# joeyee/Onet

Hardware: AMD Instinct MI355X
Metric: training images/sec (twin 256x256 pass) (higher is better)
Workload: dtype f32

## Files before the change

### onet_amd/_lib.py

```python
from __future__ import annotations

import ctypes
import os
import re

HERE = os.path.dirname(os.path.abspath(__file__))
HEADER = os.path.join(os.path.dirname(HERE), "include", "onet_hip.h")
EVAL_HEADER = os.path.join(os.path.dirname(HERE), "include", "onet_hip_eval.h")
RAGGED_HEADER = os.path.join(os.path.dirname(HERE), "include", "onet_hip_ragged.h")
RAGGED_SPLIT_HEADER = os.path.join(os.path.dirname(HERE), "include", "onet_hip_ragged_split.h")
LIBPATH = os.environ.get("ONET_HIP_LIB") or os.path.join(HERE, "libonet_hip.so")

_CT = {
    "int": ctypes.c_int,
    "int64_t": ctypes.c_int64,
    "uint64_t": ctypes.c_uint64,
    "float": ctypes.c_float,
    "double": ctypes.c_double,
}


def parse_header(path: str = HEADER):
    src = open(path).read()
    src = re.sub(r"/\*.*?\*/", " ", src, flags=re.S)
    src = re.sub(r"//[^\n]*", " ", src)
    src = re.sub(r"^\s*#.*$", " ", src, flags=re.M)
    protos = {}
    for m in re.finditer(r"((?:const\s+)?\w+\s*\*?)\s*(onet_\w+)\s*\(([^)]*)\)\s*;", src):
        ret, name, args = m.group(1).strip(), m.group(2), m.group(3).strip()
        if ret.endswith("*"):
            restype = ctypes.c_char_p if "char" in ret else ctypes.c_void_p
        else:
            restype = _CT[ret]
        argtypes, argnames = [], []
        if args and args != "void":
            for a in args.split(","):
                a = a.strip()
                mm = re.match(r"(?:const\s+)?(\w+)\s*(\*?)\s*(\w+)$", a)
                if not mm:
                    raise ValueError(f"cannot parse argument {a!r} of {name}")
                base, ptr, an = mm.groups()
                argtypes.append(ctypes.c_void_p if ptr else _CT[base])
                argnames.append(an)
        protos[name] = (restype, argtypes, argnames)
    return protos


class OnetHipError(RuntimeError):
    pass


_lib = None
_protos = None


def load(build_if_missing: bool = True):
    global _lib, _protos
    if _lib is not None:
        return _lib
    if not os.path.exists(LIBPATH):
        if not build_if_missing:
            raise OnetHipError(f"{LIBPATH} not built; run `python -m onet_amd.build`")
        from . import build as _build
        _build.build()
    lib = ctypes.CDLL(LIBPATH)
    _protos = {}
    for header in (HEADER, EVAL_HEADER, RAGGED_HEADER, RAGGED_SPLIT_HEADER):
        protos = parse_header(header)
        for name, (restype, argtypes, _) in protos.items():
            try:
                fn = getattr(lib, name)
            except AttributeError as e:
                raise OnetHipError(f"libonet_hip.so does not export {name} declared in {os.path.basename(header)}") from e
            fn.restype = restype
            fn.argtypes = argtypes
        _protos.update(protos)
    _lib = lib
    return lib


def last_error() -> str:
    return load().onet_last_error().decode()


PROFILE_HOOK = None


def call(name: str, *args, nbytes=None):
    lib = load()
    hook = PROFILE_HOOK
    tok = hook.begin() if hook is not None else None
    rc = getattr(lib, name)(*args)
    if tok is not None:
        hook.end(name, nbytes, tok)
    if rc != 0:
        raise OnetHipError(f"{name} failed ({rc}): {lib.onet_last_error().decode()}")
    return rc
```

### onet_amd/build.py

```python
import os
import subprocess
import sys

HERE = os.path.dirname(os.path.abspath(__file__))
CSRC = os.path.join(HERE, "csrc")
LIB = os.path.join(HERE, "libonet_hip.so")
SOURCES = ["abi.cpp", "conv_mfma.hip", "conv_wino4.hip", "conv_wino4w.hip", "conv_split.hip", "convt_gemm.hip", "stem.hip", "bn.hip", "spatial.hip", "head_loss.hip", "optim.hip", "evalside.hip", "clutter.hip"]
ARCH = "gfx950"


def _stale():
    if not os.path.exists(LIB):
        return True
    t = os.path.getmtime(LIB)
    deps = [os.path.join(CSRC, f) for f in os.listdir(CSRC) if f.endswith((".hip", ".cpp", ".hpp"))] + \
        [os.path.join(HERE, "..", "include", h) for h in ("onet_hip.h", "onet_hip_eval.h", "onet_hip_ragged.h", "onet_hip_ragged_split.h")]
    return any(os.path.getmtime(d) > t for d in deps)


def build(force=False, verbose=False, variant=None, flags=()):
    lib = LIB if variant is None else os.path.join(HERE, f"libonet_hip_{variant}.so")
    if variant is None and not force and not _stale():
        return LIB
    hipcc = os.environ.get("HIPCC", "/opt/rocm/bin/hipcc")
    objdir = CSRC if variant is None else os.path.join(CSRC, "_" + variant)
    os.makedirs(objdir, exist_ok=True)
    objs = []
    procs = []
    for src in SOURCES:
        obj = os.path.join(objdir, src.rsplit(".", 1)[0] + ".o")
        cmd = [hipcc, "-x", "hip", f"--offload-arch={ARCH}", "-O3", "-fPIC", "-std=c++17", "-Wall",
               "-Wno-unused-result", "-fno-slp-vectorize", *flags, "-c", os.path.join(CSRC, src), "-o", obj]
        if verbose:
            cmd.insert(-4, "-Rpass-analysis=kernel-resource-usage")
        procs.append((src, subprocess.Popen(cmd, stdout=subprocess.PIPE, stderr=subprocess.STDOUT, text=True)))
        objs.append(obj)
    failed = False
    for src, p in procs:
        out, _ = p.communicate()
        if p.returncode != 0:
            failed = True
            sys.stderr.write(f"[onet_amd.build] {src} failed:\n{out}\n")
        elif verbose or out.strip():
            sys.stderr.write(out)
    if failed:
        raise RuntimeError("hipcc failed building libonet_hip.so")
    subprocess.check_call([hipcc, "-shared", "-fPIC", f"--offload-arch={ARCH}", "-o", lib] + objs)
    return lib

# ... 8 lines not shown
```

### onet_amd/csrc/conv_split.hip

```cpp
#include <algorithm>
#include <cstdlib>
#include "common.hpp"
#include "../../include/onet_hip_ragged.h"
#include "../../include/onet_hip_ragged_split.h"

using namespace onet;

typedef float f32x16 __attribute__((ext_vector_type(16)));
typedef __bf16 bf16x8 __attribute__((ext_vector_type(8)));
typedef __bf16 bf16x2 __attribute__((ext_vector_type(2)));
typedef unsigned int u32x4s __attribute__((ext_vector_type(4)));
typedef float f32x4s __attribute__((ext_vector_type(4)));

namespace {

constexpr unsigned OOB_S = 0x80000000u;

__device__ __forceinline__ __amdgpu_buffer_rsrc_t s_rsrc(const void* base, int64_t bytes) {
    const int n = bytes > 0x7fffffffll ? 0x7fffffff : (int)bytes;
    return __builtin_amdgcn_make_buffer_rsrc(const_cast<void*>(base), 0, n, 0x00020000);
}
__device__ __forceinline__ void split2(float a, float b, unsigned& hi, unsigned& mid) {
    const bf16x2 h = {(__bf16)a, (__bf16)b};
    const bf16x2 m = {(__bf16)(a - (float)h[0]), (__bf16)(b - (float)h[1])};
    hi = __builtin_bit_cast(unsigned, h);
    mid = __builtin_bit_cast(unsigned, m);
}

typedef _Float16 f16x2 __attribute__((ext_vector_type(2)));
typedef _Float16 f16x8 __attribute__((ext_vector_type(8)));
__device__ __forceinline__ unsigned pack2bf(float lo, float hi) {
    const bf16x2 v = {(__bf16)lo, (__bf16)hi};
    return __builtin_bit_cast(unsigned, v);
}
__device__ __forceinline__ void split2h(float a, float b, unsigned& hi, unsigned& mid) {
    const f16x2 h = {(_Float16)a, (_Float16)b};
    const f16x2 m = {(_Float16)(a - (float)h[0]), (_Float16)(b - (float)h[1])};
    hi = __builtin_bit_cast(unsigned, h);
    mid = __builtin_bit_cast(unsigned, m);
}

__global__ void absmax_slots_kernel(const float* __restrict__ v, int64_t n, unsigned* __restrict__ slots) {
    float m = 0.f;
    for (int64_t i = blockIdx.x * (int64_t)blockDim.x + threadIdx.x; i < n; i += (int64_t)gridDim.x * blockDim.x) m = fmaxf(m, fabsf(v[i]));
#pragma unroll
    for (int o = 32; o > 0; o >>= 1) m = fmaxf(m, __shfl_xor(m, o, 64));
    if ((threadIdx.x & 63) == 0)
        atomicMax(slots + ((blockIdx.x * (blockDim.x >> 6) + (threadIdx.x >> 6)) & (AMAX_SLOTS - 1)) * AMAX_STRIDE, __builtin_bit_cast(unsigned, m));
}

__global__ void pack3x3_split_kernel(const float* __restrict__ w, __bf16* __restrict__ wq, int Cout, int Cin, int which, int f16,
                                     const unsigned* __restrict__ wamax) {
    const int K = which == 0 ? Cin : ((Cout + 15) / 16) * 16, N = which == 0 ? Cout : Cin;
    const int64_t n = (int64_t)K * 9 * N;
    const int nparts = f16 == 2 ? 1 : 2;
    float winv = 1.f;
    const float wscale = f16 == 1 ? amax_scale(amax_read(wamax), true, winv) : 1.f;
    if (blockIdx.x == 0 && threadIdx.x == 0) {
        float* meta = reinterpret_cast<float*>(wq + nparts * n);
        meta[0] = wscale;
        meta[1] = winv;
    }
    for (int64_t i = blockIdx.x * (int64_t)blockDim.x + threadIdx.x; i < n; i += (int64_t)gridDim.x * blockDim.x) {
        const int kc = (int)(i & 7);
        int64_t r = i >> 3;
        const int nn = (int)(r % N);
        r /= N;
        const int half = (int)(r & 1);
        r >>= 1;
        const int t = (int)(r % 9), kg = (int)(r / 9);
        const int k = kg * 16 + half * 8 + kc;
        float v = 0.f;
        if (which == 0) v = w[((int64_t)nn * Cin + k) * 9 + t];
        else if (k < Cout) v = w[((int64_t)k * Cin + nn) * 9 + (8 - t)];
        const int64_t per_chunk_part = (int64_t)9 * 2 * N * 8;
        const int64_t within = i - (int64_t)kg * per_chunk_part;
        if (f16 == 2) {
            wq[(int64_t)kg * per_chunk_part + within] = (__bf16)v;
        } else if (f16) {
            _Float16* wh = reinterpret_cast<_Float16*>(wq);
            const float vs = v * wscale;
            const _Float16 hi = (_Float16)vs;
            wh[((int64_t)kg * 2 + 0) * per_chunk_part + within] = hi;
            wh[((int64_t)kg * 2 + 1) * per_chunk_part + within] = (_Float16)(vs - (float)hi);
        } else {
            const __bf16 hi = (__bf16)v;
            wq[((int64_t)kg * 2 + 0) * per_chunk_part + within] = hi;
            wq[((int64_t)kg * 2 + 1) * per_chunk_part + within] = (__bf16)(v - (float)hi);
        }
    }
}

struct SpArgs {
    const float* x;
    int64_t x_bs;
    const __bf16* wq;
    float* z;
    int64_t z_bs;
    int B, Cin, Cout, H, W, tilesX, tilesY, coTiles;
    float* stats;
    const float* nsave;
    int nimg;
    const unsigned* x_amax;
    int x_always;
};

#define ONET_SP_DPP_ADD(v, ctrl, rmask) \
    v += __builtin_bit_cast(float, __builtin_amdgcn_update_dpp(0, __builtin_bit_cast(int, v), ctrl, rmask, 0xf, false))
__device__ __forceinline__ float sp_half_sum(float v) {
    ONET_SP_DPP_ADD(v, 0x128, 0xf);
    ONET_SP_DPP_ADD(v, 0x124, 0xf);
    ONET_SP_DPP_ADD(v, 0x122, 0xf);
    ONET_SP_DPP_ADD(v, 0x121, 0xf);
    ONET_SP_DPP_ADD(v, 0x142, 0xa);
    return v;
}
#undef ONET_SP_DPP_ADD

struct SpCfg {
    static constexpr int NW = 8, NT = 2, TW = 32, CO_T = 64;
    static constexpr int ROWS = NW * NT;
    static constexpr int IN_ROWS = ROWS + 2, IN_COLS = TW + 2;
    static constexpr int NPIX = IN_ROWS * IN_COLS;
// ... 2105 lines not shown
#undef ONET_SWP_LAUNCH
    int rc = check_launch("conv3x3_split_wgrad_pre_kernel");
    if (rc) return rc;
    return launch_wgrad_reduce((const float*)ws, dw, a.splitK * slabs, 9, Cout, Cin, 0, accumulate, as_stream(stream));
}

int onet_conv3x3_split_pack_weights(const float* w, void* wq_fwd, void* wq_dgrad, void* amax_ws, int Cout, int Cin, int fwd_f16,
                                    int dgrad_f16, void* stream) {
    ONET_REQUIRE(w && (wq_fwd || wq_dgrad), "conv3x3_split_pack_weights: null pointer");
    ONET_REQUIRE(amax_ws || !(fwd_f16 == 1 || dgrad_f16 == 1), "conv3x3_split_pack_weights: the fp16 packs need the 8 KB magnitude workspace");
    if (fwd_f16 == 1 || dgrad_f16 == 1) {
        (void)hipMemsetAsync(amax_ws, 0, AMAX_SLOTS * AMAX_STRIDE * sizeof(unsigned), as_stream(stream));
        const int64_t nw = (int64_t)Cout * Cin * 9;
        hipLaunchKernelGGL(absmax_slots_kernel, dim3((unsigned)std::min<int64_t>((nw + 1023) / 1024, 1024)), dim3(256), 0, as_stream(stream), w,
                           nw, (unsigned*)amax_ws);
        int rc0 = check_launch("absmax_slots_kernel");
        if (rc0) return rc0;
    }
    ONET_REQUIRE(Cout > 0 && Cin > 0, "conv3x3_split_pack_weights: bad shape");
    ONET_REQUIRE(!wq_fwd || (Cin % 16) == 0, "conv3x3_split_pack_weights: the forward pack needs Cin %% 16 == 0");
    const int64_t n = (int64_t)std::max(Cin, ((Cout + 15) / 16) * 16) * 9 * std::max(Cin, Cout);
    const int blocks = (int)std::min<int64_t>((n + 255) / 256, 8192);
    if (wq_fwd) {
        hipLaunchKernelGGL(pack3x3_split_kernel, dim3(blocks), dim3(256), 0, as_stream(stream), w, (__bf16*)wq_fwd, Cout, Cin, 0, fwd_f16,
                           (const unsigned*)amax_ws);
        int rc = check_launch("pack3x3_split_kernel");
        if (rc) return rc;
    }
    if (wq_dgrad) hipLaunchKernelGGL(pack3x3_split_kernel, dim3(blocks), dim3(256), 0, as_stream(stream), w, (__bf16*)wq_dgrad, Cout, Cin, 1,
                                     dgrad_f16, (const unsigned*)amax_ws);
    return check_launch("pack3x3_split_kernel");
}

int onet_conv3x3_split_fwd(const float* x, int64_t x_bs, const void* wq, int wq_f16, float* z, int64_t z_bs, int B, int Cin, int Cout,
                           int H, int W, void* stream) {
    return split_fwd(x, x_bs, wq, z, z_bs, B, Cin, Cout, H, W, stream, nullptr, wq_f16);
}

int onet_absmax_slots(const float* x, int64_t n, void* slots, void* stream) {
    ONET_REQUIRE(x && slots && n > 0, "absmax_slots: bad args");
    hipLaunchKernelGGL(absmax_slots_kernel, dim3((unsigned)std::min<int64_t>((n + 1023) / 1024, 4096)), dim3(256), 0, as_stream(stream), x, n,
                       (unsigned*)slots);
    return check_launch("absmax_slots_kernel");
}

int onet_conv3x3_split_conv_amax(const float* x, int64_t x_bs, const void* x_amax, int scale_always, const void* wq, float* z, int64_t z_bs,
                                 float* part, int B, int Cin, int Cout, int H, int W, void* stream) {
    return split_fwd(x, x_bs, wq, z, z_bs, B, Cin, Cout, H, W, stream, part, 1, nullptr, 0, (const unsigned*)x_amax, scale_always);
}

int onet_conv3x3_split_wgrad_f16(const float* x, int64_t x_bs, const void* x_amax, const float* save, int n_groups, const float* dz,
                                 int64_t dz_bs, const void* dz_amax, float* dw, void* ws, int64_t ws_bytes, int B, int Cin, int Cout,
                                 int H, int W, int accumulate, void* stream) {
    return split_wgrad_impl(x, x_bs, dz, dz_bs, dw, ws, ws_bytes, B, Cin, Cout, H, W, accumulate, stream, save, save ? n_groups : 0, 1,
                            (const unsigned*)x_amax, (const unsigned*)dz_amax);
}

int onet_conv3x3_split_fwd_norm(const float* z_prev, int64_t z_bs, const float* save, int n_groups, const void* wq, int wq_f16,
                                const void* x_amax, float* z, int64_t zo_bs, float* part, int B, int Cin, int Cout, int H, int W,
                                void* stream) {
    ONET_REQUIRE(save, "conv3x3_split_fwd_norm: null pointer");
    return split_fwd(z_prev, z_bs, wq, z, zo_bs, B, Cin, Cout, H, W, stream, part, wq_f16, save, n_groups, (const unsigned*)x_amax);
}

int onet_split_pack_act(const float* x, int64_t x_bs, void* xs, int64_t xs_bs, int B, int C, int H, int W, int f16, float scale,
                        const void* slots, void* stream) {
// ... 395 lines not shown
```

### onet_amd/csrc/convt_gemm.hip

```cpp
#include <algorithm>
#include <cstdlib>
#include "common.hpp"
#include "../../include/onet_hip_ragged.h"
#include "../../include/onet_hip_ragged_split.h"

using namespace onet;

typedef float f32x16 __attribute__((ext_vector_type(16)));
typedef float f32x4g __attribute__((ext_vector_type(4)));
typedef float f32x2g __attribute__((ext_vector_type(2)));
typedef int i32x4g __attribute__((ext_vector_type(4)));
typedef __bf16 bf16x8g __attribute__((ext_vector_type(8)));
typedef __bf16 bf16x2g __attribute__((ext_vector_type(2)));
typedef unsigned u32x4g __attribute__((ext_vector_type(4)));

namespace {

__device__ __forceinline__ i32x4g g_rsrc(const void* base, int64_t bytes) {
    const uint64_t p = reinterpret_cast<uint64_t>(base);
    i32x4g r;
    r.x = (int)(p & 0xffffffffu);
    r.y = (int)((p >> 32) & 0xffffu);
    r.z = bytes > 0x7fffffffll ? 0x7fffffff : (int)bytes;
    r.w = 0x00020000;
    return r;
}
__device__ __forceinline__ unsigned g_lds(const float* p) {
    return (unsigned)(uintptr_t)(__attribute__((address_space(3))) const float*)p;
}
__device__ __forceinline__ void g_dma16(i32x4g rsrc, unsigned lds_base, unsigned voff) {
    unsigned keep;
    asm volatile("s_nop 4\n\ts_mov_b32 %0, m0\n\ts_mov_b32 m0, %3\n\ts_nop 0\n\tbuffer_load_dwordx4 %1, %2, 0 offen lds\n\ts_mov_b32 m0, %0"
                 : "=&s"(keep)
                 : "v"(voff), "s"(rsrc), "s"(lds_base)
                 : "memory");
// ... 932 lines not shown
    }

    float undo = 1.f, dy_inv = 1.f;
    if constexpr (NP == 2) {
        float x_inv;
        (void)amax_scale(amax_read(g.x_slots), false, x_inv);
        (void)amax_scale(amax_read(g.dy_slots), true, dy_inv);
        undo = x_inv * dy_inv;
    }
    float* slab = g.slab + (int64_t)ks * g.Cin * 4 * g.Ct;
#pragma unroll
    for (int t = 0; t < TM; ++t)
#pragma unroll
        for (int u = 0; u < 2; ++u) {
            const int col = (GB * 8 * nt + chf * 32 + l31) * 4 + 2 * di + u;
#pragma unroll
            for (int r = 0; r < 16; ++r) {
                const int ci = C::MT * mt + wr * (TM * 32) + t * 32 + (r & 3) + 8 * (r >> 2) + 4 * kh;
                slab[(int64_t)ci * 4 * g.Ct + col] = acc[t][u][r] * undo;
            }
        }
    if (bias_wave && kh == 0) {
#pragma unroll
        for (int u = 0; u < 2; ++u) g.db_part[((int64_t)ks * 4 + 2 * di + u) * g.Ct + GB * 8 * nt + chf * 32 + l31] = accb[u][0] * dy_inv;
    }
}

__global__ void convt_pack_slots_kernel(const float* __restrict__ w, void* __restrict__ wP, void* __restrict__ wdP, int Cin, int Ct, int np,
                                        const unsigned* __restrict__ wamax) {
    const int M = 4 * Ct;
    const int64_t n = (int64_t)Cin * M;
    float winv = 1.f;
    const float wscale = np == 2 ? amax_scale(amax_read(wamax), true, winv) : 1.f;
    if (np == 2 && blockIdx.x == 0 && threadIdx.x == 0) {
        float* meta = reinterpret_cast<float*>(reinterpret_cast<_Float16*>(wP) + 2 * n);
        meta[0] = wscale;
        meta[1] = winv;
        if (wdP) {
            float* md = reinterpret_cast<float*>(reinterpret_cast<_Float16*>(wdP) + 2 * n);
            md[0] = wscale;
            md[1] = winv;
        }
    }
    for (int64_t i2 = blockIdx.x * (int64_t)blockDim.x + threadIdx.x; i2 < (wdP ? 2 * n : n); i2 += (int64_t)gridDim.x * blockDim.x) {
        if (i2 >= n) {
            const int64_t i = i2 - n;
            const int kc = (int)(i & 7);
            const int64_t r = i >> 3;
            const int ci = (int)(r % Cin), ks = (int)(r / Cin);
            const int c = (ks >> 2) * 8 + kc, q = ks & 3;
            const float v = w[((int64_t)ci * Ct + c) * 4 + q];
            if (np == 2) {
                _Float16* o = reinterpret_cast<_Float16*>(wdP);
                const float vs = v * wscale;
                const _Float16 hi = (_Float16)vs;
                o[(((int64_t)ks * 2 + 0) * Cin + ci) * 8 + kc] = hi;
                o[(((int64_t)ks * 2 + 1) * Cin + ci) * 8 + kc] = (_Float16)(vs - (float)hi);
            } else {
                reinterpret_cast<__bf16*>(wdP)[((int64_t)ks * Cin + ci) * 8 + kc] = (__bf16)v;
            }
            continue;
        }
        const int64_t i = i2;
        const int kc = (int)(i & 7);
        const int64_t r = i >> 3;
        const int m = (int)(r % M), c8 = (int)(r / M);
        const float v = w[(int64_t)(c8 * 8 + kc) * M + m];
        if (np == 2) {
            _Float16* o = reinterpret_cast<_Float16*>(wP);
            const float vs = v * wscale;
            const _Float16 hi = (_Float16)vs;
            o[(((int64_t)c8 * 2 + 0) * M + m) * 8 + kc] = hi;
            o[(((int64_t)c8 * 2 + 1) * M + m) * 8 + kc] = (_Float16)(vs - (float)hi);
        } else {
            reinterpret_cast<__bf16*>(wP)[((int64_t)c8 * M + m) * 8 + kc] = (__bf16)v;
        }
    }
}

__global__ void convt_absmax_kernel(const float* __restrict__ x, int64_t n, unsigned* __restrict__ slots) {
    float m = 0.f;
    for (int64_t i = blockIdx.x * (int64_t)blockDim.x + threadIdx.x; i < n; i += (int64_t)gridDim.x * blockDim.x) m = fmaxf(m, fabsf(x[i]));
#pragma unroll
    for (int o = 32; o > 0; o >>= 1) m = fmaxf(m, __shfl_xor(m, o, 64));
    if ((threadIdx.x & 63) == 0 && m == m)
        atomicMax(slots + ((blockIdx.x * (blockDim.x >> 6) + (threadIdx.x >> 6)) & (AMAX_SLOTS - 1)) * AMAX_STRIDE, __builtin_bit_cast(unsigned, m));
}

bool aligned16(const void* p) { return (reinterpret_cast<uintptr_t>(p) & 15) == 0; }

void wgrad_plan(int B, int Cin, int Ct, int h, int w, int& splitK, int& per) {
    const int64_t chunks = (int64_t)B * h * w / KP;
    const int64_t tiles = (int64_t)(Cin / 128) * (Ct / 32);
    int64_t k = std::max<int64_t>(1, (512 + tiles - 1) / tiles);
    k = std::min<int64_t>(k, std::max<int64_t>(1, chunks / 16));
    k = std::min<int64_t>(k, std::max<int64_t>(1, (256ll << 20) / ((int64_t)Cin * 4 * Ct * 4)));
    per = (int)((chunks + k - 1) / k);
    splitK = (int)((chunks + per - 1) / per);
}

}

namespace onet {


int convt_gemm_fwd(const float* x, int64_t x_bs, const float* wq, const float* bias, float* y, int64_t y_bs, void* y16, int64_t y16_bs,
                   int B, int Cin, int Ct, int h, int w, int Ho, int Wo, int pt, int pl, int prec, hipStream_t st, int y16_split,
                   const void* out_slots) {
    const int64_t hw = (int64_t)h * w;
    if (pt || pl || Ho != 2 * h || Wo != 2 * w || (Cin % KC) || (Ct % 32) || (hw % 128) || (w & 1) || !aligned16(x) || !aligned16(wq) ||
// ... 250 lines not shown
```

### onet_amd/ops.py

```python
from __future__ import annotations

import torch

from . import _lib

F32 = torch.float32


import os as _os


def _flags_from_env():
    out = {}
    for item in _os.environ.get("ONET_FLAGS", "").split(","):
        if "=" in item:
            k, v = item.split("=", 1)
            out[k.strip()] = v.strip()
    return out


_FLAGS = _flags_from_env()


def _flag(name, default):
# ... 322 lines not shown
    Cin, Cout = w.shape[0], w.shape[1]
    wq = torch.empty(Cin * 4 * Cout, dtype=F32, device=w.device)
    _lib.call("onet_convT2x2_pack_weights_fused", _p(w), _p(wq), Cin, Cout, _stream())
    return wq


CONVT_BF16 = _flag("CONVT_BF16", True)


def convT2x2_fwd(x, wq, bias, out, Ct, pt, pl):
    require_gpu(x, wq, out)
    x, xbs = plane(x)
    B, Cin, h, w = x.shape
    Ho, Wo = out.shape[2], out.shape[3]
    obs = out.stride(0) if B > 1 else Ct * Ho * Wo
    e0 = _prof_begin("convt_gemm_kernel")
    _lib.call("onet_convT2x2_fwd", _p(x), xbs, _p(wq), _p(bias), _p(out), obs, B, Cin, Ct, h, w, Ho, Wo, pt, pl,
              convt_operand_bf16(B, h, w, Ct), _stream())
    _prof_end("convt_gemm_kernel", 2.0 * B * h * w * Cin * 4 * Ct, e0, 4.0 * (B * h * w * (Cin + 4 * Ct) + 4 * Cin * Ct))


def convT2x2_out_bound(weight, bias, x_amax):
    w = weight.detach()
    w = w if w.is_contiguous() else w.contiguous()
    slots = new_amax(w.device)
    _lib.call("onet_convT2x2_out_bound", _p(w), _p(bias), w.shape[0], w.shape[1], _p(x_amax), _p(slots), _stream())
    return slots


def packT2x2_slots(w, parts=2, dgrad=False):
    require_gpu(w)
    w = w.detach().contiguous()
    Cin, Ct = w.shape[0], w.shape[1]
    dt = torch.float16 if parts == 2 else BF
    wP = torch.empty(Cin * 4 * Ct * parts + 4, dtype=dt, device=w.device)
    wdP = torch.empty(Cin * 4 * Ct * parts + 4, dtype=dt, device=w.device) if dgrad else None
    ws = torch.empty(2048, dtype=torch.int32, device=w.device) if parts == 2 else None
    _lib.call("onet_convT2x2_pack_weights_slots", _p(w), _p(wP), _p(wdP), _p(ws), Cin, Ct, parts, _stream())
    return (wP, wdP) if dgrad else wP


def convT2x2_dgrad_slots(dyP, wdP, Cin, dy_slots=None):
    B, C8, Ho, parts, Wo, _ = dyP.shape
    Ct, h, w = C8 * 8, Ho // 2, Wo // 2
    dx = torch.empty((B, Cin, h, w), dtype=F32, device=dyP.device)
    e0 = _prof_begin("convt_gemm_kernel")
    rc = _lib.load().onet_convT2x2_dgrad_slots(_p(dyP), _pbs(dyP), _p(dy_slots), _p(wdP), _p(dx), Cin * h * w, parts, B, Cin, Ct, h, w, _stream())
    flops, nb = 2.0 * B * h * w * Cin * 4 * Ct, B * h * w * (4.0 * Cin + 2.0 * parts * 4 * Ct)
    _prof_end("convt_gemm_kernel", flops if rc == 0 else 0.0, e0, nb if rc == 0 else 0.0)
    if rc < 0:
        raise _lib.OnetHipError(f"onet_convT2x2_dgrad_slots failed ({rc}): {_lib.last_error()}")
    return dx if rc == 0 else None


def convT2x2_wgrad_slots(xP, dyP, dw_shape, x_slots=None, dy_slots=None, want_dbias=False, out=None, db_out=None):
    B, C8, h, parts, w, _ = xP.shape
    Cin, Ct = C8 * 8, dyP.shape[1] * 8
    assert tuple(dw_shape) == (Cin, Ct, 2, 2) and dyP.shape[3] == parts and dyP.shape[2] == 2 * h and xP.dtype == dyP.dtype
    need = int(_lib.load().onet_convT2x2_wgrad_slots_ws_bytes(B, Cin, Ct, h, w))
    if need <= 0:
        return None
    ws = workspace(need, xP.device)
    dw = out if out is not None else torch.empty(dw_shape, dtype=F32, device=xP.device)
    db = (db_out if db_out is not None else torch.empty(Ct, dtype=F32, device=xP.device)) if want_dbias else None
    e0 = _prof_begin("convt_wgrad_gemm_kernel")
    rc = _lib.load().onet_convT2x2_wgrad_slots(_p(xP), _pbs(xP), _p(x_slots), _p(dyP), _pbs(dyP), _p(dy_slots), _p(dw), _p(db), _p(ws),
                                               ws.numel() * 4, parts, B, Cin, Ct, h, w, _stream())
    flops, nb = 2.0 * B * h * w * Cin * 4 * Ct, 2.0 * parts * B * h * w * (Cin + 4 * Ct)
    _prof_end("convt_wgrad_gemm_kernel", flops if rc == 0 else 0.0, e0, nb if rc == 0 else 0.0)
    if rc < 0:
        raise _lib.OnetHipError(f"onet_convT2x2_wgrad_slots failed ({rc}): {_lib.last_error()}")
    return (dw, db) if rc == 0 else None
# ... 419 lines not shown






def pack3x3_winograd4(w):
    require_gpu(w)
    w = w.detach().contiguous()
    Cout, Cin = w.shape[0], w.shape[1]
    wf = torch.empty(Cin * 36 * ((Cout + 63) // 64 * 64), dtype=F32, device=w.device)
    wd = torch.empty(Cout * 36 * ((Cin + 63) // 64 * 64), dtype=F32, device=w.device)
    _lib.call("onet_conv3x3_pack_weights_winograd4", _p(w), _p(wf), _p(wd), Cout, Cin, _stream())
    return wf, wd


def conv3x3_winograd4(x, wq, Cout, out=None):
    require_gpu(x, wq)
    x, xbs = plane(x)
    B, Cin, H, W = x.shape
    if out is None:
        out = torch.empty((B, Cout, H, W), dtype=F32, device=x.device)
    zbs = out.stride(0) if B > 1 else Cout * H * W
    e0 = _prof_begin("conv_wino4_kernel")
    _lib.call("onet_conv3x3_winograd4_fwd", _p(x), xbs, _p(wq), _p(out), zbs, B, Cin, Cout, H, W, _stream())
    _prof_end("conv_wino4_kernel", 2.0 * B * H * W * Cin * Cout * 9, e0, 4.0 * (B * H * W * (Cin + Cout) + 9 * Cin * Cout))
    return out


def pack3x3_plain16(w):
    require_gpu(w)
    w = w.detach().contiguous()
    Cout, Cin = w.shape[0], w.shape[1]
    wf = torch.empty(Cin * 9 * Cout + 8, dtype=BF, device=w.device) if Cin % 16 == 0 else None
    wd = torch.empty((-(-Cout // 16) * 16) * 9 * Cin + 8, dtype=BF, device=w.device)
    _lib.call("onet_conv3x3_split_pack_weights", _p(w), _p(wf), _p(wd), None, Cout, Cin, 2, 2, _stream())
    return wf, wd


def pack3x3_split(w):
    require_gpu(w)
    w = w.detach().contiguous()
    Cout, Cin = w.shape[0], w.shape[1]
    f_fwd, f_dg = split_f16(), grad_f16() or presplit()
    wf = torch.empty(2 * Cin * 9 * Cout + 8, dtype=torch.float16 if f_fwd else BF, device=w.device) if Cin % 16 == 0 else None
    wd = torch.empty(2 * (-(-Cout // 16) * 16) * 9 * Cin + 8, dtype=torch.float16 if f_dg else BF, device=w.device)
    ws = torch.empty(AMAX_SLOTS, dtype=torch.int32, device=w.device) if (f_fwd or f_dg) else None
    _lib.call("onet_conv3x3_split_pack_weights", _p(w), _p(wf), _p(wd), _p(ws), Cout, Cin, int(f_fwd), int(f_dg), _stream())
    return wf, wd


class counting_batches:

    def __enter__(self):
        self.outer = getattr(_TLS, "counters", None)
        _TLS.counters = []
        return self

    def __exit__(self, *exc):
        pending, _TLS.counters = _TLS.counters, self.outer
        by_inc = {}
        for t, n in pending:
            by_inc.setdefault(n, []).append(t)
        for n, ts in by_inc.items():
            if len(ts) > 1 and all(t.is_cuda for t in ts):
                torch._foreach_add_(ts, n)
            else:
                for t in ts:
                    t.add_(n)
        return False


def count_batches(counter, n):
    pending = getattr(_TLS, "counters", None)
    if pending is None:
        counter.add_(n)
    else:
        pending.append((counter, n))


AMAX_SLOTS = 64 * 32

# ... 1241 lines not shown
```

### onet_amd/trainer.py

```python
from __future__ import annotations

import math
import os
import time

import torch
import torch.distributed as dist

from . import ops
from .modules import invalidate_packed


def sim_lr(epoch: int, base_lr: float = 5e-6) -> float:
    return base_lr * (0.5 ** max(0, (epoch - 1) // 100)) if epoch > 0 else base_lr


def cosine_warm_restarts_lr(epoch: int, base_lr: float = 1e-4, T_0: int = 300, T_mult: int = 2,
                            eta_min: float = 1e-6) -> float:
    t, Ti = epoch, T_0
    while t >= Ti:
        t -= Ti
        Ti *= T_mult
    return eta_min + (base_lr - eta_min) * (1 + math.cos(math.pi * t / Ti)) / 2

# ... 156 lines not shown
    def _segments_with_grads(self):
        have = [p.grad is not None for p in self.params]
        if self._steps is None:
            if all(have):
                self.step_count += 1
                return [(0, self.numel, self.step_count)]
            self._steps = [self.step_count] * len(self.params)
        segs, start, cur = [], None, None
        for i, h in enumerate(have):
            if h:
                self._steps[i] += 1
            st = self._steps[i] if h else None
            if start is not None and st != cur:
                segs.append((start, self.offsets[i], cur))
                start = None
            if h and start is None:
                start, cur = self.offsets[i], st
        if start is not None:
            segs.append((start, self.numel, cur))
        self.step_count = max(self._steps)
        return segs

    def step(self):
        self._check_nan_all_ranks()
        g = self.param_groups[0]
        segs = self._segments_with_grads()
        self._gather_stray_grads()
        self.all_reduce_grads()
        for a, b, n in segs:
            ops.adam_step(self.flat[a:b], self.gflat[a:b], self.m[a:b], self.v[a:b], g["lr"], g["betas"][0], g["betas"][1],
                          g["eps"], g["weight_decay"], n, grad_scale=1.0 / self.world_size)
        torch.autograd.graph.increment_version([p for p in self.params if p.grad is not None])
        invalidate_packed(self.model)

    def broadcast_params(self, src=0):
        if self.world_size > 1 or (dist.is_available() and dist.is_initialized()):
            dist.broadcast(self.flat, src=src, group=self.pg)
            for b in self.model.buffers():
                dist.broadcast(b, src=src, group=self.pg)
            torch.autograd.graph.increment_version(self.params)
            invalidate_packed(self.model)


def init_distributed(backend: str | None = None):
    world = int(os.environ.get("WORLD_SIZE", "1"))
    rank = int(os.environ.get("RANK", "0"))
    local = int(os.environ.get("ONET_FORCE_LOCAL_RANK", os.environ.get("LOCAL_RANK", "0")))
    if "RANK" in os.environ and not dist.is_initialized():
        os.environ.setdefault("MASTER_ADDR", "127.0.0.1")
        os.environ.setdefault("MASTER_PORT", "29500")
        backend = os.environ.get("ONET_DIST_BACKEND", backend)
        if backend is None:
            backend = "nccl" if torch.cuda.is_available() else "gloo"
        if backend == "nccl":
            torch.cuda.set_device(local)
            dist.init_process_group(backend, rank=rank, world_size=world, device_id=torch.device("cuda", local))
        else:
            dist.init_process_group(backend, rank=rank, world_size=world)
    return rank, world, local


def shard_batch(X, rank: int, world: int, drop_remainder: bool = False):
    B = X.shape[0]
    if B % world:
        if not drop_remainder or B < world:
            raise ValueError(f"batch {B} not divisible by world size {world}")
        B -= B % world
    per = B // world
    return X[rank * per:(rank + 1) * per]


def train_step(onet, opt, X):
    opt.zero_grad()
    Lt, Vt, Ld, Vd, S = onet(X)
# ... 73 lines not shown
```

Before: 580.7.

## Batch all per-layer weight packing into two grouped kernels after each optimizer step

After each Adam step, all conv3x3 and transposed-conv weight packs are rebuilt through a single descriptor table. One absmax kernel and one pack kernel cover every layer, and each block finds its record by binary search, so the per-layer Python and launch sequences during the next forward go away. The cost is a pinned host table built and copied to the device every step. Packs are also produced eagerly even for layers that might not need them.

```diff
diff --git a/include/onet_hip_prep.h b/include/onet_hip_prep.h
--- /dev/null
+++ b/include/onet_hip_prep.h
@@ -0,0 +1,33 @@
+#ifndef ONET_HIP_PREP_H
+#define ONET_HIP_PREP_H
+
+#include "onet_hip.h"
+
+#ifdef __cplusplus
+extern "C" {
+#endif
+
+enum { ONET_PREP_3X3_SPLIT = 0, ONET_PREP_3X3_PLAIN16 = 1, ONET_PREP_CONVT_SLOTS = 2 };
+
+typedef struct onet_weight_prep_rec {
+    const float* w;
+    void* dst_fwd;
+    void* dst_dgrad;
+    void* slots;
+    int32_t kind;
+    int32_t Cout, Cin;
+    int32_t fwd_f16, dgrad_f16;
+    int32_t parts;
+    int32_t a_first, a_count;
+    int32_t b_first, b_fwd, b_dgrad;
+    int32_t reserved;
+} onet_weight_prep_rec;
+
+int onet_weight_prep_rec_bytes(void);
+int onet_weight_prep_plan(void* desc_host, int n, int* blocks_a, int* blocks_b);
+int onet_weight_prep_batched(const void* desc_host, const void* desc_dev, int n, void* stream);
+
+#ifdef __cplusplus
+}
+#endif
+#endif
diff --git a/onet_amd/_lib.py b/onet_amd/_lib.py
--- a/onet_amd/_lib.py
+++ b/onet_amd/_lib.py
@@ -9,6 +9,7 @@
 EVAL_HEADER = os.path.join(os.path.dirname(HERE), "include", "onet_hip_eval.h")
 RAGGED_HEADER = os.path.join(os.path.dirname(HERE), "include", "onet_hip_ragged.h")
 RAGGED_SPLIT_HEADER = os.path.join(os.path.dirname(HERE), "include", "onet_hip_ragged_split.h")
+PREP_HEADER = os.path.join(os.path.dirname(HERE), "include", "onet_hip_prep.h")
 LIBPATH = os.environ.get("ONET_HIP_LIB") or os.path.join(HERE, "libonet_hip.so")
 
 _CT = {
@@ -65,7 +66,7 @@
         _build.build()
     lib = ctypes.CDLL(LIBPATH)
     _protos = {}
-    for header in (HEADER, EVAL_HEADER, RAGGED_HEADER, RAGGED_SPLIT_HEADER):
+    for header in (HEADER, EVAL_HEADER, RAGGED_HEADER, RAGGED_SPLIT_HEADER, PREP_HEADER):
         protos = parse_header(header)
         for name, (restype, argtypes, _) in protos.items():
             try:
diff --git a/onet_amd/build.py b/onet_amd/build.py
--- a/onet_amd/build.py
+++ b/onet_amd/build.py
@@ -14,7 +14,7 @@
         return True
     t = os.path.getmtime(LIB)
     deps = [os.path.join(CSRC, f) for f in os.listdir(CSRC) if f.endswith((".hip", ".cpp", ".hpp"))] + \
-        [os.path.join(HERE, "..", "include", h) for h in ("onet_hip.h", "onet_hip_eval.h", "onet_hip_ragged.h", "onet_hip_ragged_split.h")]
+        [os.path.join(HERE, "..", "include", h) for h in ("onet_hip.h", "onet_hip_eval.h", "onet_hip_ragged.h", "onet_hip_ragged_split.h", "onet_hip_prep.h")]
     return any(os.path.getmtime(d) > t for d in deps)
 
 
diff --git a/onet_amd/csrc/conv_split.hip b/onet_amd/csrc/conv_split.hip
--- a/onet_amd/csrc/conv_split.hip
+++ b/onet_amd/csrc/conv_split.hip
@@ -1,6 +1,8 @@
 #include <algorithm>
 #include <cstdlib>
 #include "common.hpp"
+#include "weight_pack.hpp"
+#include "../../include/onet_hip_prep.h"
 #include "../../include/onet_hip_ragged.h"
 #include "../../include/onet_hip_ragged_split.h"
 
@@ -51,44 +53,128 @@
 
 __global__ void pack3x3_split_kernel(const float* __restrict__ w, __bf16* __restrict__ wq, int Cout, int Cin, int which, int f16,
                                      const unsigned* __restrict__ wamax) {
-    const int K = which == 0 ? Cin : ((Cout + 15) / 16) * 16, N = which == 0 ? Cout : Cin;
-    const int64_t n = (int64_t)K * 9 * N;
+    int N;
+    const int64_t n = pack3x3_split_geom(Cout, Cin, which, N);
     const int nparts = f16 == 2 ? 1 : 2;
     float winv = 1.f;
     const float wscale = f16 == 1 ? amax_scale(amax_read(wamax), true, winv) : 1.f;
-    if (blockIdx.x == 0 && threadIdx.x == 0) {
-        float* meta = reinterpret_cast<float*>(wq + nparts * n);
-        meta[0] = wscale;
-        meta[1] = winv;
+    if (blockIdx.x == 0 && threadIdx.x == 0) pack3x3_split_meta(wq, nparts * n, wscale, winv);
+    for (int64_t i = blockIdx.x * (int64_t)blockDim.x + threadIdx.x; i < n; i += (int64_t)gridDim.x * blockDim.x)
+        pack3x3_split_elem(w, wq, Cout, Cin, which, f16, N, wscale, i);
+}
+
+typedef onet_weight_prep_rec PrepRec;
+
+template <bool PHASE_A>
+__device__ __forceinline__ int prep_find(const PrepRec* __restrict__ tab, int n, int b) {
+    int lo = 0, hi = n - 1;
+    while (lo < hi) {
+        const int mid = (lo + hi) >> 1;
+        const int end = PHASE_A ? tab[mid].a_first + tab[mid].a_count : tab[mid].b_first + tab[mid].b_fwd + tab[mid].b_dgrad;
+        if (end > b) hi = mid;
+        else lo = mid + 1;
     }
-    for (int64_t i = blockIdx.x * (int64_t)blockDim.x + threadIdx.x; i < n; i += (int64_t)gridDim.x * blockDim.x) {
-        const int kc = (int)(i & 7);
-        int64_t r = i >> 3;
-        const int nn = (int)(r % N);
-        r /= N;
-        const int half = (int)(r & 1);
-        r >>= 1;
-        const int t = (int)(r % 9), kg = (int)(r / 9);
-        const int k = kg * 16 + half * 8 + kc;
-        float v = 0.f;
-        if (which == 0) v = w[((int64_t)nn * Cin + k) * 9 + t];
-        else if (k < Cout) v = w[((int64_t)k * Cin + nn) * 9 + (8 - t)];
-        const int64_t per_chunk_part = (int64_t)9 * 2 * N * 8;
-        const int64_t within = i - (int64_t)kg * per_chunk_part;
-        if (f16 == 2) {
-            wq[(int64_t)kg * per_chunk_part + within] = (__bf16)v;
-        } else if (f16) {
-            _Float16* wh = reinterpret_cast<_Float16*>(wq);
-            const float vs = v * wscale;
-            const _Float16 hi = (_Float16)vs;
-            wh[((int64_t)kg * 2 + 0) * per_chunk_part + within] = hi;
-            wh[((int64_t)kg * 2 + 1) * per_chunk_part + within] = (_Float16)(vs - (float)hi);
+    return lo;
+}
+
+__global__ void weight_prep_absmax_kernel(const PrepRec* __restrict__ tab, int n) {
+    const PrepRec r = tab[prep_find<true>(tab, n, (int)blockIdx.x)];
+    const int lb = (int)blockIdx.x - r.a_first, nb = r.a_count;
+    if (lb < 0 || lb >= nb) return;
+    const int64_t nw = r.kind == ONET_PREP_CONVT_SLOTS ? (int64_t)r.Cin * 4 * r.Cout : (int64_t)r.Cout * r.Cin * 9;
+    const float* __restrict__ w = r.w;
+    float m = 0.f;
+    for (int64_t i = lb * (int64_t)blockDim.x + threadIdx.x; i < nw; i += (int64_t)nb * blockDim.x) m = fmaxf(m, fabsf(w[i]));
+#pragma unroll
+    for (int o = 32; o > 0; o >>= 1) m = fmaxf(m, __shfl_xor(m, o, 64));
+    if ((threadIdx.x & 63) == 0 && (r.kind != ONET_PREP_CONVT_SLOTS || m == m))
+        atomicMax(reinterpret_cast<unsigned*>(r.slots) + ((lb * (blockDim.x >> 6) + (threadIdx.x >> 6)) & (AMAX_SLOTS - 1)) * AMAX_STRIDE,
+                  __builtin_bit_cast(unsigned, m));
+}
+
+__global__ void weight_prep_pack_kernel(const PrepRec* __restrict__ tab, int n) {
+    const PrepRec r = tab[prep_find<false>(tab, n, (int)blockIdx.x)];
+    int lb = (int)blockIdx.x - r.b_first;
+    if (lb < 0 || lb >= r.b_fwd + r.b_dgrad) return;
+    const unsigned* wamax = reinterpret_cast<const unsigned*>(r.slots);
+    float winv = 1.f;
+    if (r.kind == ONET_PREP_CONVT_SLOTS) {
+        const int64_t nc = (int64_t)r.Cin * 4 * r.Cout;
+        const int nb = r.b_fwd;
+        const float wscale = r.parts == 2 ? amax_scale(amax_read(wamax), true, winv) : 1.f;
+        if (r.parts == 2 && lb == 0 && threadIdx.x == 0) convt_pack_slots_meta(r.dst_fwd, r.dst_dgrad, nc, wscale, winv);
+        for (int64_t i2 = lb * (int64_t)blockDim.x + threadIdx.x; i2 < (r.dst_dgrad ? 2 * nc : nc); i2 += (int64_t)nb * blockDim.x)
+            convt_pack_slots_elem(r.w, r.dst_fwd, r.dst_dgrad, r.Cin, r.Cout, r.parts, wscale, nc, i2);
+        return;
+    }
+    const int which = lb >= r.b_fwd ? 1 : 0;
+    const int nb = which ? r.b_dgrad : r.b_fwd;
+    if (which) lb -= r.b_fwd;
+    const int f16 = r.kind == ONET_PREP_3X3_PLAIN16 ? 2 : (which ? r.dgrad_f16 : r.fwd_f16);
+    __bf16* wq = reinterpret_cast<__bf16*>(which ? r.dst_dgrad : r.dst_fwd);
+    int N;
+    const int64_t n1 = pack3x3_split_geom(r.Cout, r.Cin, which, N);
+    const float wscale = f16 == 1 ? amax_scale(amax_read(wamax), true, winv) : 1.f;
+    if (lb == 0 && threadIdx.x == 0) pack3x3_split_meta(wq, (f16 == 2 ? 1 : 2) * n1, wscale, winv);
+    for (int64_t i = lb * (int64_t)blockDim.x + threadIdx.x; i < n1; i += (int64_t)nb * blockDim.x)
+        pack3x3_split_elem(r.w, wq, r.Cout, r.Cin, which, f16, N, wscale, i);
+}
+
+constexpr int PREP_BLOCK_ELEMS = 2048;
+
+bool prep_aligned(const void* p, uintptr_t a) { return (reinterpret_cast<uintptr_t>(p) & (a - 1)) == 0; }
+
+int prep_check(PrepRec* tab, int n, bool fill, int* blocks_a, int* blocks_b) {
+    ONET_REQUIRE(tab, "weight_prep: null table");
+    ONET_REQUIRE(n > 0, "weight_prep: bad record count %d", n);
+    int64_t ta = 0, tb = 0;
+    int stale = -1;
+    for (int i = 0; i < n; ++i) {
+        const PrepRec& r = tab[i];
+        ONET_REQUIRE(r.kind == ONET_PREP_3X3_SPLIT || r.kind == ONET_PREP_3X3_PLAIN16 || r.kind == ONET_PREP_CONVT_SLOTS,
+                     "weight_prep: record %d: unknown kind %d", i, r.kind);
+        ONET_REQUIRE(r.w, "weight_prep: record %d: null weight pointer", i);
+        ONET_REQUIRE(r.Cout > 0 && r.Cin > 0, "weight_prep: record %d: bad shape", i);
+        bool f16;
+        int64_t nw, nf = 0, nd = 0;
+        if (r.kind == ONET_PREP_CONVT_SLOTS) {
+            ONET_REQUIRE(r.dst_fwd, "weight_prep: record %d: null forward pack", i);
+            ONET_REQUIRE(r.parts == 1 || r.parts == 2, "weight_prep: record %d: bad number of parts %d", i, r.parts);
+            ONET_REQUIRE((r.Cin % 8) == 0 && (!r.dst_dgrad || (r.Cout % 8) == 0),
+                         "weight_prep: record %d: the slot packs need Cin %% 8 == 0 (and Ct %% 8 == 0 for the input gradient's)", i);
+            f16 = r.parts == 2;
+            nw = (int64_t)r.Cin * 4 * r.Cout;
+            nf = (r.dst_dgrad ? 2 : 1) * nw;
         } else {
-            const __bf16 hi = (__bf16)v;
-            wq[((int64_t)kg * 2 + 0) * per_chunk_part + within] = hi;
-            wq[((int64_t)kg * 2 + 1) * per_chunk_part + within] = (__bf16)(v - (float)hi);
-        }
+            ONET_REQUIRE(r.dst_fwd || r.dst_dgrad, "weight_prep: record %d: null pack pointers", i);
+            ONET_REQUIRE(!r.dst_fwd || (r.Cin % 16) == 0, "weight_prep: record %d: the forward pack needs Cin %% 16 == 0", i);
+            const bool split = r.kind == ONET_PREP_3X3_SPLIT;
+            ONET_REQUIRE(!split || ((r.fwd_f16 == 0 || r.fwd_f16 == 1) && (r.dgrad_f16 == 0 || r.dgrad_f16 == 1)),
+                         "weight_prep: record %d: bad part formats", i);
+            f16 = split && ((r.dst_fwd && r.fwd_f16 == 1) || (r.dst_dgrad && r.dgrad_f16 == 1));
+            nw = (int64_t)r.Cout * r.Cin * 9;
+            if (r.dst_fwd) nf = nw;
+            if (r.dst_dgrad) nd = (int64_t)((r.Cout + 15) / 16 * 16) * 9 * r.Cin;
+        }
+        ONET_REQUIRE(!f16 || r.slots, "weight_prep: record %d: the fp16 packs need the 8 KB magnitude slots", i);
+        ONET_REQUIRE(prep_aligned(r.w, 4) && prep_aligned(r.slots, 4) && prep_aligned(r.dst_fwd, 16) && prep_aligned(r.dst_dgrad, 16),
+                     "weight_prep: record %d: pointer not aligned (weight and slots: 4 bytes, packs: 16)", i);
+        const int64_t ca = f16 ? std::min<int64_t>((nw + 1023) / 1024, 1024) : 0;
+        const int64_t cf = (nf + PREP_BLOCK_ELEMS - 1) / PREP_BLOCK_ELEMS, cd = (nd + PREP_BLOCK_ELEMS - 1) / PREP_BLOCK_ELEMS;
+        ONET_REQUIRE(ta + ca < (1ll << 30) && tb + cf + cd < (1ll << 30), "weight_prep: grid too large at record %d", i);
+        if (fill) {
+            tab[i].a_first = (int32_t)ta, tab[i].a_count = (int32_t)ca;
+            tab[i].b_first = (int32_t)tb, tab[i].b_fwd = (int32_t)cf, tab[i].b_dgrad = (int32_t)cd;
+        } else if (stale < 0 && !(r.a_first == ta && r.a_count == ca && r.b_first == tb && r.b_fwd == cf && r.b_dgrad == cd)) {
+            stale = i;
+        }
+        ta += ca;
+        tb += cf + cd;
     }
+    ONET_REQUIRE(stale < 0, "weight_prep: record %d: block ranges are not onet_weight_prep_plan's", stale);
+    *blocks_a = (int)ta;
+    *blocks_b = (int)tb;
+    return ONET_OK;
 }
 
 struct SpArgs {
@@ -2260,6 +2346,32 @@
     return check_launch("pack3x3_split_kernel");
 }
 
+int onet_weight_prep_rec_bytes(void) { return (int)sizeof(onet_weight_prep_rec); }
+
+int onet_weight_prep_plan(void* desc_host, int n, int* blocks_a, int* blocks_b) {
+    int ta = 0, tb = 0;
+    int rc = prep_check(static_cast<PrepRec*>(desc_host), n, true, &ta, &tb);
+    if (rc) return rc;
+    if (blocks_a) *blocks_a = ta;
+    if (blocks_b) *blocks_b = tb;
+    return ONET_OK;
+}
+
+int onet_weight_prep_batched(const void* desc_host, const void* desc_dev, int n, void* stream) {
+    int ta = 0, tb = 0;
+    int rc = prep_check(const_cast<PrepRec*>(static_cast<const PrepRec*>(desc_host)), n, false, &ta, &tb);
+    if (rc) return rc;
+    ONET_REQUIRE(desc_dev && prep_aligned(desc_dev, 8), "weight_prep: null or misaligned device table");
+    const PrepRec* tab = static_cast<const PrepRec*>(desc_dev);
+    if (ta > 0) {
+        hipLaunchKernelGGL(weight_prep_absmax_kernel, dim3((unsigned)ta), dim3(256), 0, as_stream(stream), tab, n);
+        rc = check_launch("weight_prep_absmax_kernel");
+        if (rc) return rc;
+    }
+    hipLaunchKernelGGL(weight_prep_pack_kernel, dim3((unsigned)tb), dim3(256), 0, as_stream(stream), tab, n);
+    return check_launch("weight_prep_pack_kernel");
+}
+
 int onet_conv3x3_split_fwd(const float* x, int64_t x_bs, const void* wq, int wq_f16, float* z, int64_t z_bs, int B, int Cin, int Cout,
                            int H, int W, void* stream) {
     return split_fwd(x, x_bs, wq, z, z_bs, B, Cin, Cout, H, W, stream, nullptr, wq_f16);
diff --git a/onet_amd/csrc/convt_gemm.hip b/onet_amd/csrc/convt_gemm.hip
--- a/onet_amd/csrc/convt_gemm.hip
+++ b/onet_amd/csrc/convt_gemm.hip
@@ -1,6 +1,7 @@
 #include <algorithm>
 #include <cstdlib>
 #include "common.hpp"
+#include "weight_pack.hpp"
 #include "../../include/onet_hip_ragged.h"
 #include "../../include/onet_hip_ragged_split.h"
 
@@ -999,50 +1000,9 @@
     const int64_t n = (int64_t)Cin * M;
     float winv = 1.f;
     const float wscale = np == 2 ? amax_scale(amax_read(wamax), true, winv) : 1.f;
-    if (np == 2 && blockIdx.x == 0 && threadIdx.x == 0) {
-        float* meta = reinterpret_cast<float*>(reinterpret_cast<_Float16*>(wP) + 2 * n);
-        meta[0] = wscale;
-        meta[1] = winv;
-        if (wdP) {
-            float* md = reinterpret_cast<float*>(reinterpret_cast<_Float16*>(wdP) + 2 * n);
-            md[0] = wscale;
-            md[1] = winv;
-        }
-    }
-    for (int64_t i2 = blockIdx.x * (int64_t)blockDim.x + threadIdx.x; i2 < (wdP ? 2 * n : n); i2 += (int64_t)gridDim.x * blockDim.x) {
-        if (i2 >= n) {
-            const int64_t i = i2 - n;
-            const int kc = (int)(i & 7);
-            const int64_t r = i >> 3;
-            const int ci = (int)(r % Cin), ks = (int)(r / Cin);
-            const int c = (ks >> 2) * 8 + kc, q = ks & 3;
-            const float v = w[((int64_t)ci * Ct + c) * 4 + q];
-            if (np == 2) {
-                _Float16* o = reinterpret_cast<_Float16*>(wdP);
-                const float vs = v * wscale;
-                const _Float16 hi = (_Float16)vs;
-                o[(((int64_t)ks * 2 + 0) * Cin + ci) * 8 + kc] = hi;
-                o[(((int64_t)ks * 2 + 1) * Cin + ci) * 8 + kc] = (_Float16)(vs - (float)hi);
-            } else {
-                reinterpret_cast<__bf16*>(wdP)[((int64_t)ks * Cin + ci) * 8 + kc] = (__bf16)v;
-            }
-            continue;
-        }
-        const int64_t i = i2;
-        const int kc = (int)(i & 7);
-        const int64_t r = i >> 3;
-        const int m = (int)(r % M), c8 = (int)(r / M);
-        const float v = w[(int64_t)(c8 * 8 + kc) * M + m];
-        if (np == 2) {
-            _Float16* o = reinterpret_cast<_Float16*>(wP);
-            const float vs = v * wscale;
-            const _Float16 hi = (_Float16)vs;
-            o[(((int64_t)c8 * 2 + 0) * M + m) * 8 + kc] = hi;
-            o[(((int64_t)c8 * 2 + 1) * M + m) * 8 + kc] = (_Float16)(vs - (float)hi);
-        } else {
-            reinterpret_cast<__bf16*>(wP)[((int64_t)c8 * M + m) * 8 + kc] = (__bf16)v;
-        }
-    }
+    if (np == 2 && blockIdx.x == 0 && threadIdx.x == 0) convt_pack_slots_meta(wP, wdP, n, wscale, winv);
+    for (int64_t i2 = blockIdx.x * (int64_t)blockDim.x + threadIdx.x; i2 < (wdP ? 2 * n : n); i2 += (int64_t)gridDim.x * blockDim.x)
+        convt_pack_slots_elem(w, wP, wdP, Cin, Ct, np, wscale, n, i2);
 }
 
 __global__ void convt_absmax_kernel(const float* __restrict__ x, int64_t n, unsigned* __restrict__ slots) {
diff --git a/onet_amd/csrc/weight_pack.hpp b/onet_amd/csrc/weight_pack.hpp
--- /dev/null
+++ b/onet_amd/csrc/weight_pack.hpp
@@ -0,0 +1,93 @@
+#pragma once
+#include "common.hpp"
+
+namespace onet {
+
+__device__ __forceinline__ int64_t pack3x3_split_geom(int Cout, int Cin, int which, int& N) {
+    const int K = which == 0 ? Cin : ((Cout + 15) / 16) * 16;
+    N = which == 0 ? Cout : Cin;
+    return (int64_t)K * 9 * N;
+}
+__device__ __forceinline__ void pack3x3_split_meta(__bf16* wq, int64_t n_all, float wscale, float winv) {
+    float* meta = reinterpret_cast<float*>(wq + n_all);
+    meta[0] = wscale;
+    meta[1] = winv;
+}
+__device__ __forceinline__ void pack3x3_split_elem(const float* w, __bf16* wq, int Cout, int Cin, int which, int f16,
+                                                   int N, float wscale, int64_t i) {
+    const int kc = (int)(i & 7);
+    int64_t r = i >> 3;
+    const int nn = (int)(r % N);
+    r /= N;
+    const int half = (int)(r & 1);
+    r >>= 1;
+    const int t = (int)(r % 9), kg = (int)(r / 9);
+    const int k = kg * 16 + half * 8 + kc;
+    float v = 0.f;
+    if (which == 0) v = w[((int64_t)nn * Cin + k) * 9 + t];
+    else if (k < Cout) v = w[((int64_t)k * Cin + nn) * 9 + (8 - t)];
+    const int64_t per_chunk_part = (int64_t)9 * 2 * N * 8;
+    const int64_t within = i - (int64_t)kg * per_chunk_part;
+    if (f16 == 2) {
+        wq[(int64_t)kg * per_chunk_part + within] = (__bf16)v;
+    } else if (f16) {
+        _Float16* wh = reinterpret_cast<_Float16*>(wq);
+        const float vs = v * wscale;
+        const _Float16 hi = (_Float16)vs;
+        wh[((int64_t)kg * 2 + 0) * per_chunk_part + within] = hi;
+        wh[((int64_t)kg * 2 + 1) * per_chunk_part + within] = (_Float16)(vs - (float)hi);
+    } else {
+        const __bf16 hi = (__bf16)v;
+        wq[((int64_t)kg * 2 + 0) * per_chunk_part + within] = hi;
+        wq[((int64_t)kg * 2 + 1) * per_chunk_part + within] = (__bf16)(v - (float)hi);
+    }
+}
+
+__device__ __forceinline__ void convt_pack_slots_meta(void* wP, void* wdP, int64_t n, float wscale, float winv) {
+    float* meta = reinterpret_cast<float*>(reinterpret_cast<_Float16*>(wP) + 2 * n);
+    meta[0] = wscale;
+    meta[1] = winv;
+    if (wdP) {
+        float* md = reinterpret_cast<float*>(reinterpret_cast<_Float16*>(wdP) + 2 * n);
+        md[0] = wscale;
+        md[1] = winv;
+    }
+}
+__device__ __forceinline__ void convt_pack_slots_elem(const float* w, void* wP, void* wdP, int Cin, int Ct,
+                                                      int np, float wscale, int64_t n, int64_t i2) {
+    const int M = 4 * Ct;
+    if (i2 >= n) {
+        const int64_t i = i2 - n;
+        const int kc = (int)(i & 7);
+        const int64_t r = i >> 3;
+        const int ci = (int)(r % Cin), ks = (int)(r / Cin);
+        const int c = (ks >> 2) * 8 + kc, q = ks & 3;
+        const float v = w[((int64_t)ci * Ct + c) * 4 + q];
+        if (np == 2) {
+            _Float16* o = reinterpret_cast<_Float16*>(wdP);
+            const float vs = v * wscale;
+            const _Float16 hi = (_Float16)vs;
+            o[(((int64_t)ks * 2 + 0) * Cin + ci) * 8 + kc] = hi;
+            o[(((int64_t)ks * 2 + 1) * Cin + ci) * 8 + kc] = (_Float16)(vs - (float)hi);
+        } else {
+            reinterpret_cast<__bf16*>(wdP)[((int64_t)ks * Cin + ci) * 8 + kc] = (__bf16)v;
+        }
+        return;
+    }
+    const int64_t i = i2;
+    const int kc = (int)(i & 7);
+    const int64_t r = i >> 3;
+    const int m = (int)(r % M), c8 = (int)(r / M);
+    const float v = w[(int64_t)(c8 * 8 + kc) * M + m];
+    if (np == 2) {
+        _Float16* o = reinterpret_cast<_Float16*>(wP);
+        const float vs = v * wscale;
+        const _Float16 hi = (_Float16)vs;
+        o[(((int64_t)c8 * 2 + 0) * M + m) * 8 + kc] = hi;
+        o[(((int64_t)c8 * 2 + 1) * M + m) * 8 + kc] = (_Float16)(vs - (float)hi);
+    } else {
+        reinterpret_cast<__bf16*>(wP)[((int64_t)c8 * M + m) * 8 + kc] = (__bf16)v;
+    }
+}
+
+}
diff --git a/onet_amd/ops.py b/onet_amd/ops.py
--- a/onet_amd/ops.py
+++ b/onet_amd/ops.py
@@ -378,12 +378,18 @@
     require_gpu(w)
     w = w.detach().contiguous()
     Cin, Ct = w.shape[0], w.shape[1]
-    dt = torch.float16 if parts == 2 else BF
-    wP = torch.empty(Cin * 4 * Ct * parts + 4, dtype=dt, device=w.device)
-    wdP = torch.empty(Cin * 4 * Ct * parts + 4, dtype=dt, device=w.device) if dgrad else None
+    wP, wdP = _allocT_slots(w, parts, dgrad)
     ws = torch.empty(2048, dtype=torch.int32, device=w.device) if parts == 2 else None
     _lib.call("onet_convT2x2_pack_weights_slots", _p(w), _p(wP), _p(wdP), _p(ws), Cin, Ct, parts, _stream())
     return (wP, wdP) if dgrad else wP
+
+
+def _allocT_slots(w, parts, dgrad):
+    Cin, Ct = w.shape[0], w.shape[1]
+    dt = torch.float16 if parts == 2 else torch.bfloat16
+    wP = torch.empty(Cin * 4 * Ct * parts + 4, dtype=dt, device=w.device)
+    wdP = torch.empty(Cin * 4 * Ct * parts + 4, dtype=dt, device=w.device) if dgrad else None
+    return wP, wdP
 
 
 def convT2x2_dgrad_slots(dyP, wdP, Cin, dy_slots=None):
@@ -869,9 +875,15 @@
     require_gpu(w)
     w = w.detach().contiguous()
     Cout, Cin = w.shape[0], w.shape[1]
+    wf, wd = _alloc3x3_plain16(w)
+    _lib.call("onet_conv3x3_split_pack_weights", _p(w), _p(wf), _p(wd), None, Cout, Cin, 2, 2, _stream())
+    return wf, wd
+
+
+def _alloc3x3_plain16(w):
+    Cout, Cin = w.shape[0], w.shape[1]
     wf = torch.empty(Cin * 9 * Cout + 8, dtype=BF, device=w.device) if Cin % 16 == 0 else None
     wd = torch.empty((-(-Cout // 16) * 16) * 9 * Cin + 8, dtype=BF, device=w.device)
-    _lib.call("onet_conv3x3_split_pack_weights", _p(w), _p(wf), _p(wd), None, Cout, Cin, 2, 2, _stream())
     return wf, wd
 
 
@@ -879,12 +891,110 @@
     require_gpu(w)
     w = w.detach().contiguous()
     Cout, Cin = w.shape[0], w.shape[1]
-    f_fwd, f_dg = split_f16(), grad_f16() or presplit()
-    wf = torch.empty(2 * Cin * 9 * Cout + 8, dtype=torch.float16 if f_fwd else BF, device=w.device) if Cin % 16 == 0 else None
-    wd = torch.empty(2 * (-(-Cout // 16) * 16) * 9 * Cin + 8, dtype=torch.float16 if f_dg else BF, device=w.device)
+    f_fwd, f_dg = _split_pack_formats()
+    wf, wd = _alloc3x3_split(w, f_fwd, f_dg)
     ws = torch.empty(AMAX_SLOTS, dtype=torch.int32, device=w.device) if (f_fwd or f_dg) else None
     _lib.call("onet_conv3x3_split_pack_weights", _p(w), _p(wf), _p(wd), _p(ws), Cout, Cin, int(f_fwd), int(f_dg), _stream())
     return wf, wd
+
+
+def _split_pack_formats():
+    return bool(split_f16()), bool(grad_f16() or presplit())
+
+
+def _alloc3x3_split(w, f_fwd, f_dg):
+    Cout, Cin = w.shape[0], w.shape[1]
+    wf = torch.empty(2 * Cin * 9 * Cout + 8, dtype=torch.float16 if f_fwd else BF, device=w.device) if Cin % 16 == 0 else None
+    wd = torch.empty(2 * (-(-Cout // 16) * 16) * 9 * Cin + 8, dtype=torch.float16 if f_dg else BF, device=w.device)
+    return wf, wd
+
+
+WEIGHT_PREP = _flag("WEIGHT_PREP", True)
+
+import ctypes as _ctypes
+
+
+class _PrepRec(_ctypes.Structure):
+    _fields_ = [("w", _ctypes.c_void_p), ("dst_fwd", _ctypes.c_void_p), ("dst_dgrad", _ctypes.c_void_p), ("slots", _ctypes.c_void_p),
+                ("kind", _ctypes.c_int32), ("Cout", _ctypes.c_int32), ("Cin", _ctypes.c_int32), ("fwd_f16", _ctypes.c_int32),
+                ("dgrad_f16", _ctypes.c_int32), ("parts", _ctypes.c_int32), ("a_first", _ctypes.c_int32), ("a_count", _ctypes.c_int32),
+                ("b_first", _ctypes.c_int32), ("b_fwd", _ctypes.c_int32), ("b_dgrad", _ctypes.c_int32), ("reserved", _ctypes.c_int32)]
+
+
+PREP_3X3_SPLIT, PREP_3X3_PLAIN16, PREP_CONVT_SLOTS = 0, 1, 2
+
+
+def weight_prep_batched(records, device):
+    lib = _lib.load()
+    if lib.onet_weight_prep_rec_bytes() != _ctypes.sizeof(_PrepRec):
+        raise _lib.OnetHipError("onet_weight_prep_rec: the library's record size differs from ops._PrepRec")
+    n, size = len(records), _ctypes.sizeof(_PrepRec)
+    host = torch.zeros(n * size, dtype=torch.uint8, pin_memory=True)
+    tab = (_PrepRec * n).from_address(host.data_ptr())
+    for r, d in zip(tab, records):
+        r.w, r.dst_fwd, r.dst_dgrad, r.slots = _p(d["w"]), _p(d.get("dst_fwd")), _p(d.get("dst_dgrad")), _p(d.get("slots"))
+        r.kind, r.Cout, r.Cin = d["kind"], d["Cout"], d["Cin"]
+        r.fwd_f16, r.dgrad_f16, r.parts = int(d.get("fwd_f16", 0)), int(d.get("dgrad_f16", 0)), int(d.get("parts", 0))
+    if lib.onet_weight_prep_plan(host.data_ptr(), n, None, None) != 0:
+        raise _lib.OnetHipError(f"onet_weight_prep_plan failed: {_lib.last_error()}")
+    dev = host.to(device, non_blocking=True)
+    _lib.call("onet_weight_prep_batched", host.data_ptr(), _p(dev), n, _stream())
+
+
+def prepare_weight_packs(model):
+    if not WEIGHT_PREP:
+        return 0
+    from .modules import _Packable
+    todo, records, device = [], [], None
+    with torch.no_grad(), using(getattr(model, "settings", None)):
+        fmt = _split_pack_formats()
+        for m in model.modules():
+            old = getattr(m, "_pack", None)
+            w = getattr(m, "weight", None)
+            if not isinstance(m, _Packable) or old is None or w is None or not w.is_cuda or w.dtype != F32 or not w.is_contiguous():
+                continue
+            if device is None:
+                device = w.device
+            if w.device != device:
+                continue
+            wd_ = w.detach()
+            recs = []
+            if isinstance(old, Packed3x3):
+                new = Packed3x3(w)
+                Cout, Cin = w.shape[0], w.shape[1]
+                for algo in ("split", "plain16"):
+                    have = old.get(algo)
+                    if have is None:
+                        continue
+                    if algo == "split":
+                        if tuple(p.dtype == torch.float16 for p in have if p is not None) != tuple(f for f, p in zip(fmt, have) if p is not None):
+                            continue
+                        wf, wdg = _alloc3x3_split(w, *fmt)
+                        need = fmt[1] or (fmt[0] and wf is not None)
+                        recs.append(dict(kind=PREP_3X3_SPLIT, w=wd_, dst_fwd=wf, dst_dgrad=wdg, Cout=Cout, Cin=Cin, fwd_f16=fmt[0], dgrad_f16=fmt[1],
+                                         slots=new_amax(w.device) if need else None))
+                    else:
+                        wf, wdg = _alloc3x3_plain16(w)
+                        recs.append(dict(kind=PREP_3X3_PLAIN16, w=wd_, dst_fwd=wf, dst_dgrad=wdg, Cout=Cout, Cin=Cin))
+                    new[algo] = (wf, wdg)
+            elif isinstance(old, PackedT):
+                new = PackedT(w)
+                for parts, have in old._s.items():
+                    wP, wdP = _allocT_slots(w, parts, isinstance(have, tuple))
+                    recs.append(dict(kind=PREP_CONVT_SLOTS, w=wd_, dst_fwd=wP, dst_dgrad=wdP, Cout=w.shape[1], Cin=w.shape[0], parts=parts,
+                                     slots=new_amax(w.device) if parts == 2 else None))
+                    new._s[parts] = (wP, wdP) if wdP is not None else wP
+            else:
+                continue
+            if recs:
+                records += recs
+                todo.append((m, new, (w.data_ptr(), w._version, str(w.device))))
+        if not records:
+            return 0
+        weight_prep_batched(records, device)
+    for m, new, key in todo:
+        m._pack, m._pack_key = new, key
+    return len(todo)
 
 
 class counting_batches:
diff --git a/onet_amd/trainer.py b/onet_amd/trainer.py
--- a/onet_amd/trainer.py
+++ b/onet_amd/trainer.py
@@ -212,6 +212,7 @@
                           g["eps"], g["weight_decay"], n, grad_scale=1.0 / self.world_size)
         torch.autograd.graph.increment_version([p for p in self.params if p.grad is not None])
         invalidate_packed(self.model)
+        ops.prepare_weight_packs(self.model)
 
     def broadcast_params(self, src=0):
         if self.world_size > 1 or (dist.is_available() and dist.is_initialized()):
@@ -220,6 +221,7 @@
                 dist.broadcast(b, src=src, group=self.pg)
             torch.autograd.graph.increment_version(self.params)
             invalidate_packed(self.model)
+            ops.prepare_weight_packs(self.model)
 
 
 def init_distributed(backend: str | None = None):
```

Result: no change. 583.1 (median of 6 runs) (+0.4%).
